# semihkacmaz/CoNFiLD

Measured on AMD Instinct MI355X. Metric: generated fields/sec (256-step sample + CNF decode), Case4 latent, 1/2/4/8 GPU, higher is better.
Workload: dtype f32

## Files before the change

confild_amd/csrc/siren.hip:

```cpp
#include <cmath>
#include <algorithm>
#include <cstdlib>
#include <cstring>
#include <string>
#include <type_traits>
#include <utility>
#include <vector>

#include "siren.hpp"

namespace cfd {

template <int NB, bool DUAL, int WAVES>
__global__ __launch_bounds__(64 * WAVES, (NB <= 24 && !DUAL) ? 2 : 1) void siren_fused(SirenArgs p) {
    constexpr int TILE = 16 * WAVES;
    constexpr int H = NB * 16;
    constexpr int BLK = NB * 256;
    extern __shared__ __attribute__((aligned(16))) float smem[];
    float* wbuf = smem;
    float* film = smem + 2 * BLK;

    const int lane = threadIdx.x & 63;
    const int wave = threadIdx.x >> 6;
    const int g = lane >> 4;
// ... 924 lines not shown
        case 12: return launch_siren_nb<12>(h, a, b, st);
        case 16: return launch_siren_nb<16>(h, a, b, st);
        case 24: return launch_siren_nb<24>(h, a, b, st);
        case 32: return launch_siren_nb<32>(h, a, b, st);
        default: throw cfd::Error{CFD_EARG, "hidden_features must be 16*{1,2,3,4,6,8,12,16,24,32}"};
    }
}

}

namespace {

void pack_split_f16(cfd_siren* h, int li, const float* W) {
    const int H = h->cfg.hidden_features, NB = h->NB, NQ = NB / 2;
    float amax = 0.f;
    for (size_t i = 0; i < (size_t)H * H; ++i) amax = std::max(amax, std::fabs(W[i]));
    int e = 0;
    if (amax > 0.f) std::frexp(amax, &e);
    const float s = std::ldexp(1.0f, -e);
    std::vector<_Float16> img((size_t)NB * NB * 512);
    for (int j = 0; j < NB; ++j)
        for (int q = 0; q < NQ; ++q)
            for (int l = 0; l < 64; ++l)
                for (int t = 0; t < 8; ++t) {
                    const float v = W[(size_t)(16 * j + l % 16) * H + 16 * (2 * q + t / 4) + 4 * (l / 16) + t % 4] * s;
                    const _Float16 hi = (_Float16)v;
                    const _Float16 lo = (_Float16)(v - (float)hi);
                    const size_t base = ((size_t)j * NB + 2 * q) * 512 + l * 8 + t;
                    img[base] = hi;
                    img[base + 512] = lo;
                }
    CFD_HIP(hipMemcpy(h->wimg16 + (size_t)(li - 1) * NB * NB * 256, img.data(), img.size() * sizeof(_Float16),
                      hipMemcpyHostToDevice));
    for (int j = 0; j < NB; ++j)
        for (int q = 0; q < NQ; ++q)
            for (int l = 0; l < 64; ++l)
                for (int t = 0; t < 8; ++t) {
                    const float v = W[(size_t)(16 * (2 * q + t / 4) + 4 * (l / 16) + t % 4) * H + 16 * j + l % 16] * s;
                    const _Float16 hi = (_Float16)v;
                    const _Float16 lo = (_Float16)(v - (float)hi);
                    const size_t base = ((size_t)j * NB + 2 * q) * 512 + l * 8 + t;
                    img[base] = hi;
                    img[base + 512] = lo;
                }
    CFD_HIP(hipMemcpy(h->wimg16t + (size_t)(h->cfg.num_hidden_layers - li) * NB * NB * 256, img.data(),
                      img.size() * sizeof(_Float16), hipMemcpyHostToDevice));
    if (H % 32 == 0) {
        const int NB2 = H / 32, NK = H / 16;
        for (int J = 0; J < NB2; ++J)
            for (int k = 0; k < NK; ++k)
                for (int l = 0; l < 64; ++l)
                    for (int t = 0; t < 8; ++t) {
                        const int jb = k / 2, e = k % 2;
                        const float v = W[(size_t)(32 * J + l % 32) * H + 32 * jb + 8 * (2 * e + t / 4) +
                                          4 * (l / 32) + t % 4] * s;
                        const _Float16 hi = (_Float16)v;
                        const _Float16 lo = (_Float16)(v - (float)hi);
                        const size_t base = ((size_t)J * NK + k) * 1024 + l * 8 + t;
                        img[base] = hi;
                        img[base + 512] = lo;
                    }
        CFD_HIP(hipMemcpy(h->wimg32 + (size_t)(li - 1) * NB * NB * 256, img.data(),
                          img.size() * sizeof(_Float16), hipMemcpyHostToDevice));
        const double kr = (double)h->cfg.w0 / (2.0 * M_PI);
        const double amr = (double)amax * kr;
        int er = 0;
        if (amr > 0.0) std::frexp(amr, &er);
        const double sr = std::ldexp(1.0, -er);
        for (int J = 0; J < NB2; ++J)
            for (int k = 0; k < NK; ++k)
                for (int l = 0; l < 64; ++l)
                    for (int t = 0; t < 8; ++t) {
                        const int jb = k / 2, e = k % 2;
                        const double v = (double)W[(size_t)(32 * J + l % 32) * H + 32 * jb + 8 * (2 * e + t / 4) +
                                                   4 * (l / 32) + t % 4] * kr * sr;
                        const _Float16 hi = (_Float16)v;
                        const _Float16 lo = (_Float16)(v - (double)hi);
                        const size_t base = ((size_t)J * NK + k) * 1024 + l * 8 + t;
                        img[base] = hi;
                        img[base + 512] = lo;
                    }
        CFD_HIP(hipMemcpy(h->wimg32r + (size_t)(li - 1) * NB * NB * 256, img.data(),
                          img.size() * sizeof(_Float16), hipMemcpyHostToDevice));
        const int nh = h->cfg.num_hidden_layers;
        const float fs = (float)(kr * sr), inv = (float)(1.0 / sr);
        CFD_HIP(hipMemcpy(h->wrev + (li - 1), &fs, sizeof(float), hipMemcpyHostToDevice));
        CFD_HIP(hipMemcpy(h->wrev + nh + (li - 1), &inv, sizeof(float), hipMemcpyHostToDevice));
    }
    CFD_HIP(hipMemcpy(h->wscale + (li - 1), &s, sizeof(float), hipMemcpyHostToDevice));
}

}

extern "C" int cfd_siren_create(const cfd_siren_cfg* cfg, int device, cfd_siren** out) {
    return cfd::guard([&] {
        CFD_REQUIRE(cfg && out, CFD_EARG, "null argument");
        const int d = cfg->in_coord_features, L = cfg->in_latent_features, c = cfg->out_features;
        const int nh = cfg->num_hidden_layers, H = cfg->hidden_features;
        CFD_REQUIRE(d >= 1 && d <= 4, CFD_EARG, "in_coord_features must be 1..4");
        CFD_REQUIRE(c >= 1 && c <= 4, CFD_EARG, "out_features must be 1..4");
        CFD_REQUIRE(L >= 1 && nh >= 0 && H % 16 == 0 && H >= 16 && H <= 512, CFD_EARG,
                    "hidden_features must be a multiple of 16 in [16, 512]");
        const int NB = H / 16;
        CFD_REQUIRE(NB == 1 || NB == 2 || NB == 3 || NB == 4 || NB == 6 || NB == 8 || NB == 12 || NB == 16 ||
                        NB == 24 || NB == 32,
                    CFD_EARG, "hidden_features must be 16*{1,2,3,4,6,8,12,16,24,32}");
        cfd::DeviceGuard dg(device);
        auto* h = new cfd_siren();
        h->cfg = *cfg;
        if (h->cfg.w0 == 0.f) h->cfg.w0 = 30.f;
        h->device = device;
        h->NB = NB;
        for (int i = 0; i < nh + 2; ++i) {
            const int fin = i == 0 ? d : H, fout = i == nh + 1 ? c : H;
            h->params.push_back({"net1." + std::to_string(i) + ".weight", {fout, fin}});
            h->params.push_back({"net1." + std::to_string(i) + ".bias", {fout}});
        }
        for (int i = 0; i < nh + 1; ++i) h->params.push_back({"net2." + std::to_string(i) + ".weight", {H, L}});
        CFD_HIP(hipMalloc(&h->w0, sizeof(float) * H * d));
        CFD_HIP(hipMalloc(&h->fbias, sizeof(float) * (nh + 1) * H));
        CFD_HIP(hipMalloc(&h->V, sizeof(float) * (size_t)(nh + 1) * H * L));
        CFD_HIP(hipMalloc(&h->wimg, sizeof(float) * (size_t)std::max(nh, 1) * NB * NB * 256));
        CFD_HIP(hipMalloc(&h->wout, sizeof(float) * c * H));
        CFD_HIP(hipMalloc(&h->bout, sizeof(float) * 4));
        CFD_HIP(hipMalloc(&h->wimg_t, sizeof(float) * (size_t)std::max(nh, 1) * NB * NB * 256));
        CFD_HIP(hipMalloc(&h->wimg16, sizeof(float) * (size_t)std::max(nh, 1) * NB * NB * 256));
        CFD_HIP(hipMalloc(&h->wimg16t, sizeof(float) * (size_t)std::max(nh, 1) * NB * NB * 256));
        CFD_HIP(hipMalloc(&h->wscale, sizeof(float) * (size_t)std::max(nh, 1)));
        CFD_HIP(hipMalloc(&h->wimg32, sizeof(float) * (size_t)std::max(nh, 1) * NB * NB * 256));
        CFD_HIP(hipMalloc(&h->wimg32r, sizeof(float) * (size_t)std::max(nh, 1) * NB * NB * 256));
        CFD_HIP(hipMalloc(&h->wrev, sizeof(float) * 2 * (size_t)std::max(nh, 1)));
        *out = h;
    });
}

extern "C" void cfd_siren_destroy(cfd_siren* h) {
    if (!h) return;
    (void)hipFree(h->w0);
    (void)hipFree(h->fbias);
    (void)hipFree(h->V);
    (void)hipFree(h->wimg);
    (void)hipFree(h->wout);
    (void)hipFree(h->bout);
    (void)hipFree(h->wimg_t);
    (void)hipFree(h->wimg16);
    (void)hipFree(h->wimg16t);
    (void)hipFree(h->wscale);
    (void)hipFree(h->wimg32);
    (void)hipFree(h->wimg32r);
    (void)hipFree(h->wrev);
    delete h;
}

extern "C" int cfd_siren_num_params(const cfd_siren* h, int* n) {
    return cfd::guard([&] {
        CFD_REQUIRE(h && n, CFD_EARG, "null argument");
        *n = (int)h->params.size();
    });
}

extern "C" int cfd_siren_param_info(const cfd_siren* h, int idx, const char** key, int* ndim, int64_t shape[4]) {
    return cfd::guard([&] {
        CFD_REQUIRE(h && idx >= 0 && idx < (int)h->params.size(), CFD_EARG, "bad index");
        const auto& p = h->params[idx];
        if (key) *key = p.key.c_str();
        if (ndim) *ndim = (int)p.shape.size();
        if (shape)
            for (size_t i = 0; i < p.shape.size(); ++i) shape[i] = p.shape[i];
    });
}

extern "C" int cfd_siren_set_param(cfd_siren* h, const char* key, const float* host, size_t n) {
    return cfd::guard([&] {
        CFD_REQUIRE(h && key && host, CFD_EARG, "null argument");
        cfd::DeviceGuard dg(h->device);
        const std::string k(key);
        cfd::SirenParam* prm = nullptr;
        for (auto& p : h->params)
            if (p.key == k) prm = &p;
        CFD_REQUIRE(prm, CFD_EKEY, "unknown SIREN parameter key: " + k);
        size_t want = 1;
        for (auto s : prm->shape) want *= (size_t)s;
        CFD_REQUIRE(n == want, CFD_ESHAPE, "size mismatch for " + k);
        const int d = h->cfg.in_coord_features, L = h->cfg.in_latent_features, c = h->cfg.out_features;
        const int nh = h->cfg.num_hidden_layers, H = h->cfg.hidden_features, NB = h->NB;
        const bool is_w = k.size() > 7 && k.compare(k.size() - 7, 7, ".weight") == 0;
        const int li = std::stoi(k.substr(5, k.find('.', 5) - 5));
        if (k.rfind("net2.", 0) == 0) {
            CFD_HIP(hipMemcpy(h->V + (size_t)li * H * L, host, n * 4, hipMemcpyHostToDevice));
        } else if (li == nh + 1) {
            CFD_HIP(hipMemcpy(is_w ? h->wout : h->bout, host, n * 4, hipMemcpyHostToDevice));
        } else if (!is_w) {
            CFD_HIP(hipMemcpy(h->fbias + (size_t)li * H, host, n * 4, hipMemcpyHostToDevice));
        } else if (li == 0) {
            CFD_HIP(hipMemcpy(h->w0, host, n * 4, hipMemcpyHostToDevice));
            (void)d;
        } else {
            std::vector<float> img((size_t)NB * NB * 256);
            for (int j = 0; j < NB; ++j)
                for (int q = 0; q < NB; ++q)
                    for (int lane = 0; lane < 64; ++lane)
                        for (int s = 0; s < 4; ++s)
                            img[(((size_t)j * NB + q) * 64 + lane) * 4 + s] =
                                host[(size_t)(16 * j + (lane & 15)) * H + 16 * q + 4 * (lane >> 4) + s];
            CFD_HIP(hipMemcpy(h->wimg + (size_t)(li - 1) * NB * NB * 256, img.data(), img.size() * 4,
                              hipMemcpyHostToDevice));
            for (int j = 0; j < NB; ++j)
                for (int q = 0; q < NB; ++q)
                    for (int lane = 0; lane < 64; ++lane)
                        for (int s2 = 0; s2 < 4; ++s2)
                            img[(((size_t)j * NB + q) * 64 + lane) * 4 + s2] =
                                host[(size_t)(16 * q + 4 * (lane >> 4) + s2) * H + 16 * j + (lane & 15)];
            CFD_HIP(hipMemcpy(h->wimg_t + (size_t)(nh - li) * NB * NB * 256, img.data(), img.size() * 4,
                              hipMemcpyHostToDevice));
            if (NB % 2 == 0) pack_split_f16(h, li, host);
        }
        (void)c;
        prm->set = true;
    });
}

extern "C" int cfd_siren_ready(const cfd_siren* h) {
    return cfd::guard([&] {
        CFD_REQUIRE(h, CFD_EARG, "null handle");
        for (const auto& p : h->params) CFD_REQUIRE(p.set, CFD_ESTATE, "SIREN parameter not set: " + p.key);
    });
}

extern "C" int cfd_siren_workspace_bytes(const cfd_siren* h, int b, size_t* bytes) {
    return cfd::guard([&] {
        CFD_REQUIRE(h && bytes && b >= 0, CFD_EARG, "bad argument");
        *bytes = sizeof(float) * (size_t)b * (h->cfg.num_hidden_layers + 1) * h->cfg.hidden_features;
    });
}

namespace cfd {
void film_vectors(const cfd_siren* h, const float* latents, int b, float* film, hipStream_t st) {
    const int nl = h->cfg.num_hidden_layers + 1, H = h->cfg.hidden_features, L = h->cfg.in_latent_features;
    if (L % 16 == 0) {
        cfd::launch_gemm_f32(true, latents, L, h->V, L, h->fbias, film, nl * H, b, nl * H, L, st);
        return;
    }
    hipLaunchKernelGGL(cfd::siren_film, dim3(nl, b), dim3(128), 0, st, h->V, h->fbias, latents, film, H, L, nl);
    cfd::check_launch("siren_film");
}
}
using cfd::film_vectors;

extern "C" int cfd_siren_forward(cfd_siren* h, const float* coords, int64_t N, const float* latents, int b,
                                 const float* xmax, const float* xmin, const float* ymax, const float* ymin,
                                 int64_t y_stride, float* out, void* ws, size_t ws_bytes, void* stream) {
    return cfd::guard([&] {
        CFD_REQUIRE(h && coords && latents && out, CFD_EARG, "null argument");
        CFD_REQUIRE(N >= 1 && b >= 1, CFD_EARG, "empty decode");
        CFD_REQUIRE((xmax == nullptr) == (xmin == nullptr), CFD_EARG, "xmax/xmin must both be set or both NULL");
        CFD_REQUIRE((ymax == nullptr) == (ymin == nullptr), CFD_EARG, "ymax/ymin must both be set or both NULL");
        size_t need = 0;
        cfd_siren_workspace_bytes(h, b, &need);
        CFD_REQUIRE(ws && ws_bytes >= need, CFD_EARG, "workspace too small");
        const int nh = h->cfg.num_hidden_layers, H = h->cfg.hidden_features;
        auto st = (hipStream_t)stream;
        float* film = (float*)ws;
        film_vectors(h, latents, b, film, st);
        cfd::SirenArgs a{};
        a.w0 = h->w0;
        a.wimg = h->wimg;
        a.wout = h->wout;
        a.bout = h->bout;
        a.film = film;
        a.coords = coords;
        a.xmax = xmax;
        a.xmin = xmin;
        a.ymax = ymax;
        a.ymin = ymin;
        a.out = out;
        a.N = N;
        a.ystride = y_stride;
        a.d = h->cfg.in_coord_features;
        a.c = h->cfg.out_features;
        a.nh = nh;
        a.stamps = cfd::stamps_buf();
        a.w0f = h->cfg.w0;
        if (h->compute == CFD_SIREN_SPLIT_F16 && nh >= 1 && cfd::siren_split_supported(h->NB)) {
            a.wscale = h->wscale;
            if (cfd::siren_split32_supported(H, nh)) {
                a.wimg = h->wimg32;
                a.wimg_rev = h->wimg32r;
                a.wrev = h->wrev;
                cfd::launch_siren_split32(H, a, b, st);
            } else {
                a.wimg = h->wimg16;
                cfd::launch_siren_split(h->NB, a, b, st);
            }
        } else {
            launch_siren(h, a, b, st);
        }
    });
}

extern "C" int cfd_siren_set_compute(cfd_siren* h, int compute) {
    return cfd::guard([&] {
        CFD_REQUIRE(h, CFD_EARG, "null handle");
        CFD_REQUIRE(compute == CFD_SIREN_F32 || compute == CFD_SIREN_SPLIT_F16, CFD_EARG, "unknown SIREN compute mode");
        h->compute = compute;
    });
}

extern "C" int cfd_siren_get_compute(const cfd_siren* h, int* compute) {
    return cfd::guard([&] {
        CFD_REQUIRE(h && compute, CFD_EARG, "null argument");
        const bool split = h->compute == CFD_SIREN_SPLIT_F16 && h->cfg.num_hidden_layers >= 1 &&
                           cfd::siren_split_supported(h->NB);
        *compute = split ? CFD_SIREN_SPLIT_F16 : CFD_SIREN_F32;
    });
}

namespace {

void tape_args(const cfd_siren* h, cfd::SirenTapeArgs& a, int64_t Ns, int R, void* ws) {
    const int nh = h->cfg.num_hidden_layers, H = h->cfg.hidden_features;
    const size_t nl = nh + 1;
    a.w0 = h->w0;
    a.wimg = h->wimg;
    a.wimg_t = h->wimg_t;
    a.wout = h->wout;
    a.bout = h->bout;
    a.film = (float*)ws;
    a.u = (float*)ws + (size_t)R * nl * H;
    a.delta = a.u + (size_t)R * Ns * nl * H;
    a.P = (int64_t)R * Ns;
    a.Ns = (int)Ns;
    a.d = h->cfg.in_coord_features;
    a.c = h->cfg.out_features;
    a.nh = nh;
    a.w0f = h->cfg.w0;
    if (h->compute == CFD_SIREN_SPLIT_F16 && nh >= 1 && cfd::tape_split_supported(h->NB)) {
        a.wimg16 = h->wimg16;
        a.wimg16t = h->wimg16t;
        a.wscale = h->wscale;
    }
}

int tape_waves(int64_t P) { return P >= 16 * 4 * 512 ? 4 : P >= 16 * 2 * 256 ? 2 : 1; }

template <int NB, int W>
void launch_tape_w(const cfd::SirenTapeArgs& a, bool bwd, hipStream_t st) {
    const size_t lds = sizeof(float) * (2 * NB * 256 + (bwd ? 0 : 4 * NB * 16));
    const void* fn = bwd ? (const void*)cfd::siren_tape_bwd<NB, W> : (const void*)cfd::siren_tape_fwd<NB, W>;
    CFD_HIP(hipFuncSetAttribute(fn, hipFuncAttributeMaxDynamicSharedMemorySize, (int)lds));
    const dim3 grid((unsigned)cfd::ceil_div(a.P, 16 * W));
    if (bwd)
        hipLaunchKernelGGL((cfd::siren_tape_bwd<NB, W>), grid, dim3(64 * W), lds, st, a);
    else
        hipLaunchKernelGGL((cfd::siren_tape_fwd<NB, W>), grid, dim3(64 * W), lds, st, a);
    cfd::check_launch(bwd ? "siren_tape_bwd" : "siren_tape_fwd");
}

template <int NB, int KS>
void launch_tape_ks(const cfd::SirenTapeArgs& a, bool bwd, hipStream_t st) {
    const size_t lds = sizeof(float) * (2 * NB * 256 + 2 * KS * 256 + (bwd ? 0 : 4 * NB * 16 + KS * 64));
    const void* fn = bwd ? (const void*)cfd::siren_tape_bwd_ks<NB, KS> : (const void*)cfd::siren_tape_fwd_ks<NB, KS>;
    CFD_HIP(hipFuncSetAttribute(fn, hipFuncAttributeMaxDynamicSharedMemorySize, (int)lds));
    const dim3 grid((unsigned)cfd::ceil_div(a.P, 16));
    if (bwd)
        hipLaunchKernelGGL((cfd::siren_tape_bwd_ks<NB, KS>), grid, dim3(64 * KS), lds, st, a);
    else
        hipLaunchKernelGGL((cfd::siren_tape_fwd_ks<NB, KS>), grid, dim3(64 * KS), lds, st, a);
    cfd::check_launch(bwd ? "siren_tape_bwd_ks" : "siren_tape_fwd_ks");
}

// ... 243 lines not shown
```

confild_amd/csrc/siren.hpp:

```cpp
#pragma once
#include <string>
#include <type_traits>
#include <utility>
#include <vector>

#include "common.hpp"

namespace cfd {

template <int N, class F, int... I>
__device__ __forceinline__ void static_for_impl(F&& f, std::integer_sequence<int, I...>) {
    (f(std::integral_constant<int, I>{}), ...);
}
template <int N, class F>
__device__ __forceinline__ void static_for(F&& f) {
    static_for_impl<N>(f, std::make_integer_sequence<int, N>{});
}

struct SirenArgs {
    const float* w0;
    const float* wimg;
    const float* wout;
    const float* bout;
    const float* film;
    const float* coords;
    const float* xmax;
    const float* xmin;
    const float* ymax;
    const float* ymin;
    float* out;
    const float* wscale;
    const float* wimg_rev;
    const float* wrev;
    int64_t N;
    int64_t ystride;
    int64_t b0;
    int d, c, nh;
    float w0f;
    unsigned long long* stamps;
};
struct SirenTapeArgs {
    const float* w0;
    const float* wimg;
    const float* wimg_t;
    const float* wout;
    const float* bout;
    const float* film;
    const float* coords;
    const float* xmax;
    const float* xmin;
    const float* ymax;
    const float* ymin;
    float* u;
    float* delta;
    float* out;
    const float* gout;
    const float* wimg16;
    const float* wimg16t;
    const float* wscale;
    int64_t P;
    int64_t ystride;
    int Ns, d, c, nh;
    float w0f;
};
unsigned long long* stamps_buf();

template <int NB, int WAVES>
__device__ __forceinline__ void siren_issue_block(const float* __restrict__ wimg, int J, float* dst,
                                                  int wave, int lane) {
    constexpr int BLK = NB * 256;
    const float* src = wimg + (int64_t)__builtin_amdgcn_readfirstlane(J) * BLK;
    for (int piece = wave; piece < NB; piece += WAVES) {
        __builtin_amdgcn_global_load_lds((const void*)(src + piece * 256 + lane * 4),
                                         (__attribute__((address_space(3))) void*)(dst + piece * 256),
                                         16, 0, 0);
    }
}

template <int NB, int WAVES>
__device__ __forceinline__ void siren_issue_block_u(const float* __restrict__ wimg, int J, float* dst,
                                                    int wave, int lane) {
    static_assert(NB % WAVES == 0, "whole pieces per wave");
    constexpr int BLK = NB * 256;
    const float* src = wimg + (int64_t)__builtin_amdgcn_readfirstlane(J) * BLK;
    static_for<NB / WAVES>([&](auto mc) {
        constexpr int m = decltype(mc)::value;
        const int piece = wave + m * WAVES;
        __builtin_amdgcn_global_load_lds((const void*)(src + piece * 256 + lane * 4),
                                         (__attribute__((address_space(3))) void*)(dst + piece * 256), 16, 0, 0);
    });
}

bool siren_split_supported(int NB);
void launch_siren_split(int NB, SirenArgs a, int b, hipStream_t st);
bool siren_split32_supported(int H, int nh);
void launch_siren_split32(int H, SirenArgs a, int b, hipStream_t st);
bool tape_split_supported(int NB);
void launch_tape_split(int NB, const SirenTapeArgs& a, bool bwd, hipStream_t st);
void launch_tape_split_sum(int NB, const SirenTapeArgs& a, int rows, hipStream_t st);

struct SirenParam {
    std::string key;
    std::vector<int64_t> shape;
    bool set = false;
};

}

struct cfd_siren {
    cfd_siren_cfg cfg;
    int device = 0;
    int NB = 0;
    std::vector<cfd::SirenParam> params;
    float* w0 = nullptr;
    float* fbias = nullptr;
    float* V = nullptr;
    float* wimg = nullptr;
    float* wout = nullptr;
    float* bout = nullptr;
    float* wimg_t = nullptr;
    float* wimg16 = nullptr;
    float* wimg16t = nullptr;
    float* wscale = nullptr;
    float* wimg32 = nullptr;
    float* wimg32r = nullptr;
    float* wrev = nullptr;
    int compute = CFD_SIREN_SPLIT_F16;
    int dense_bwd = CFD_DENSE_BWD_SUM;
    int dense_compute = CFD_DENSE_COMPUTE_AUTO;
};

namespace cfd {

int gemm_splits(int K);
void launch_gemm_f32(bool bt, const float* A, int lda, const float* B, int ldb, const float* bias, float* C, int ldc,
                     int M, int N, int K, hipStream_t st, float* part = nullptr);
void film_vectors(const cfd_siren* h, const float* latents, int b, float* film, hipStream_t st);

}
```

confild_amd/csrc/siren_split.hip:

```cpp
#include <cstdint>
#include <cstdlib>
#include <algorithm>

#include "siren.hpp"

typedef _Float16 h8 __attribute__((ext_vector_type(8)));
typedef _Float16 h2 __attribute__((ext_vector_type(2)));
typedef float f2 __attribute__((ext_vector_type(2)));
typedef unsigned u2 __attribute__((ext_vector_type(2)));
typedef unsigned u4 __attribute__((ext_vector_type(4)));

namespace cfd {

struct Frag {
    u4 v;
    __device__ __forceinline__ h8 h() const { return __builtin_bit_cast(h8, v); }
};

__device__ __forceinline__ unsigned pk_f16(float a, float b) {
    return __builtin_bit_cast(unsigned, __builtin_convertvector((f2){a, b}, h2));
}

__device__ __forceinline__ void split8(const float (&x0)[4], const float (&x1)[4], Frag& hi, Frag& lo) {
    unsigned hw[4], lw[4];
// ... 252 lines not shown
                for (int c = 0; c < CG; ++c)
                    a[c] = __builtin_amdgcn_mfma_f32_16x16x32_f16(FL[q], BH[c][q].h(), a[c], 0, 0, 0);
#pragma unroll
                for (int c = 0; c < CG; ++c)
                    a[c] = __builtin_amdgcn_mfma_f32_16x16x32_f16(FH[q], BL[c][q].h(), a[c], 0, 0, 0);
#pragma unroll
                for (int c = 0; c < CG; ++c)
                    a[c] = __builtin_amdgcn_mfma_f32_16x16x32_f16(FH[q], BH[c][q].h(), a[c], 0, 0, 0);
                if constexpr (j > 0) {
                    if constexpr (q == 0) sines(prev);
                    if constexpr (q == QE) epilogue(std::integral_constant<int, j - 1>{});
                }
                __builtin_amdgcn_sched_barrier(0);
            });
#pragma unroll
            for (int c = 0; c < CG; ++c) prev[c] = a[c];
            if constexpr (j % RB == RB - 1) {
                if (NOSYNC) {
                } else if (steady) {
                    if (PC_HI == PC_LO || !pc_hi)
                        __builtin_amdgcn_s_waitcnt(vmcnt_imm((RING - 2) * PC_LO));
                    else
                        __builtin_amdgcn_s_waitcnt(vmcnt_imm((RING - 2) * PC_HI));
                } else {
                    __builtin_amdgcn_s_waitcnt(vmcnt_imm(0));
                }
                if (!NOSYNC) asm volatile("s_barrier" ::: "memory");
                ++J;
                slot = slot == RING - 1 ? 0 : slot + 1;
            }
        });
        sines(prev);
        epilogue(std::integral_constant<int, NB - 1>{});
        static_for<NQ>([&](auto qc) {
            constexpr int q = decltype(qc)::value;
#pragma unroll
            for (int c = 0; c < CG; ++c) {
                BH[c][q] = NH[c][q];
                BL[c][q] = NL[c][q];
            }
        });
    }

#pragma unroll
    for (int c = 0; c < CG; ++c) {
        float ov[4];
#pragma unroll
        for (int oc = 0; oc < 4; ++oc) {
            float sum = o[c][oc];
            sum += __shfl_xor(sum, 16);
            sum += __shfl_xor(sum, 32);
            ov[oc] = oc < p.c ? sum + p.bout[oc] : 0.f;
        }
        const int64_t n = n0 + 16 * c;
        if (n < p.N && g < p.c) {
            float v = g == 0 ? ov[0] : g == 1 ? ov[1] : g == 2 ? ov[2] : ov[3];
            if (p.ymax) {
                const int64_t yi = n * p.ystride + g;
                const float hi = p.ymax[yi], lo = p.ymin[yi];
                v = (v + 1.0f) / 2.0f * (hi - lo) + lo;
            }
            p.out[(b * p.N + n) * p.c + g] = v;
        }
    }
}

typedef float f16v __attribute__((ext_vector_type(16)));

__device__ __forceinline__ void split2_mix(float a, float b, unsigned& hi, unsigned& lo) {
    hi = pk_f16(a, b);
    asm("v_fma_mixlo_f16 %0, %1, 1.0, -%2 op_sel_hi:[0,0,1]" : "=&v"(lo) : "v"(a), "v"(hi));
    asm("v_fma_mixhi_f16 %0, %1, 1.0, -%2 op_sel:[0,0,1] op_sel_hi:[0,0,1]" : "+v"(lo) : "v"(b), "v"(hi));
}

__device__ __forceinline__ void split_chunk(const float (&x)[16], int e, Frag& hi, Frag& lo) {
    unsigned hw[4], lw[4];
#pragma unroll
    for (int w = 0; w < 4; ++w) split2_mix(x[8 * e + 2 * w], x[8 * e + 2 * w + 1], hw[w], lw[w]);
    hi.v = (u4){hw[0], hw[1], hw[2], hw[3]};
    lo.v = (u4){lw[0], lw[1], lw[2], lw[3]};
    asm volatile("" : "+v"(hi.v), "+v"(lo.v));
}

template <int NB2, int EXP = 0, int HWSIN = 0>
__global__ __launch_bounds__(256, 1) void siren_split32(SirenArgs p) {
    constexpr int NK = 2 * NB2;
    constexpr int H = 32 * NB2;
    constexpr int BLK = NK * 512;
    constexpr int WAVES = 4, TILE = 128;
    constexpr int NPC = 2 * NK;
    constexpr int PPW = NPC / WAVES;
    constexpr int NKS = NK >= 18 ? 16 : NK - 2;
    extern __shared__ __attribute__((aligned(16))) float smem[];
    const int nh = p.nh;
    float* wbuf = smem;
    float* film = smem + 2 * BLK;
    float* w0s = film + (nh + 1) * H;
    float* wos = w0s + 4 * H;

    const int lane = threadIdx.x & 63;
    const int wave = __builtin_amdgcn_readfirstlane(threadIdx.x >> 6);
    const int h = lane >> 5;
    const int64_t b = p.b0 + blockIdx.y;
    const int64_t n = (int64_t)blockIdx.x * TILE + wave * 32 + (lane & 31);
    CFD_DASSERT(p.d >= 1 && p.d <= 4 && p.c >= 1 && p.c <= 4 && nh >= 1);
#ifdef CFD_STAMPS
    const bool stamped = blockIdx.x % 61 == 0;
    if (stamped) CFD_STAMP(p.stamps, 5, (unsigned)blockIdx.y, 0);
    __builtin_amdgcn_s_waitcnt(0xC07F);
#endif

    {
        const float* fsrc = p.film + b * (int64_t)(nh + 1) * H;
        const int nf = (nh + 1) * H;
        for (int i = threadIdx.x * 4; i < nf; i += 64 * WAVES * 4) {
            const int layer = i / H;
            const float sc = layer == 0 ? 1.0f : HWSIN >= 3 ? p.wrev[layer - 1] : p.wscale[layer - 1];
            *(f4*)(film + i) = *(const f4*)(fsrc + i) * sc;
        }
    }
    for (int f = threadIdx.x; f < H; f += 64 * WAVES) {
        f4 w = {0.f, 0.f, 0.f, 0.f};
        for (int k = 0; k < p.d; ++k) w[k] = p.w0[f * p.d + k];
        *(f4*)(w0s + 4 * f) = w;
    }
    for (int i = threadIdx.x; i < 4 * H; i += 64 * WAVES) wos[i] = i < p.c * H ? p.wout[i] : 0.f;
    float cn[4];
    {
        const int64_t nc = n < p.N ? n : p.N - 1;
#pragma unroll
        for (int k = 0; k < 4; ++k) {
            float v = 0.f;
            if (k < p.d) {
                v = p.coords[nc * p.d + k];
                if (p.xmax) v = (v - p.xmin[k]) / (p.xmax[k] - p.xmin[k]) * 2.0f - 1.0f;
            }
            cn[k] = v;
        }
    }
    __syncthreads();
    const int nblocks = nh * NB2;
    const __amdgpu_buffer_rsrc_t wrsrc =
        __builtin_amdgcn_make_buffer_rsrc((void*)p.wimg, 0, nblocks * (BLK * 4), 0x00020000);
    siren_issue_block<NPC, WAVES>(p.wimg, 0, wbuf, wave, lane);

    Frag BH[NK], BL[NK], NH[NK], NL[NK];
    float o[4] = {0.f, 0.f, 0.f, 0.f};

    static_for<NB2>([&](auto Jc) {
        constexpr int J = decltype(Jc)::value;
        float x[16];
#pragma unroll
        for (int qq = 0; qq < 4; ++qq) {
            const f4 fv = *(const f4*)(film + 32 * J + 8 * qq + 4 * h);
#pragma unroll
            for (int r = 0; r < 4; ++r) {
                const f4 w = *(const f4*)(w0s + 4 * (32 * J + 8 * qq + 4 * h + r));
                float a = cn[0] * w[0];
#pragma unroll
                for (int k = 1; k < 4; ++k)
                    if (k < p.d) a = fmaf(cn[k], w[k], a);
                x[4 * qq + r] = hidden_sine<HWSIN >= 2 ? 2 : HWSIN>(p.w0f * (a + fv[r]));
            }
        }
        split_chunk(x, 0, NH[2 * J], NL[2 * J]);
        split_chunk(x, 1, NH[2 * J + 1], NL[2 * J + 1]);
    });

    static_assert(NB2 % 2 == 0, "static ring slots need an even block count");
    int J = 0;
    f16v prev;
    float mprev = 0.f;
    float x[16];
    h8 FH, FL;
    f16v an;
    auto film_row = [&](const float* frow) __attribute__((always_inline)) {
#pragma unroll
        for (int qq = 0; qq < 4; ++qq) {
            const f4 f = *(const f4*)(frow + 8 * qq + 4 * h);
#pragma unroll
            for (int r = 0; r < 4; ++r) an[4 * qq + r] = f[r];
        }
    };
    if constexpr (!(EXP & 1)) {
        __builtin_amdgcn_s_waitcnt(vmcnt_imm(0));
        asm volatile("s_barrier" ::: "memory");
    }
    FH = *(const h8*)(wbuf + lane * 4);
    FL = *(const h8*)(wbuf + 256 + lane * 4);
    for (int layer = 1; layer <= nh; ++layer) {
        const bool last = layer == nh;
        const float m = HWSIN >= 3 ? p.wrev[nh + layer - 1] : p.w0f / p.wscale[layer - 1];
        auto outsum = [&](int jp, int e) __attribute__((always_inline)) {
            const int f = 32 * jp + 8 * e + 4 * h;
#pragma unroll
            for (int oc = 0; oc < 4; ++oc) {
                const f4 w = *(const f4*)(wos + oc * H + f);
#pragma unroll
                for (int r = 0; r < 4; ++r) o[oc] = fmaf(w[r], x[4 * e + r], o[oc]);
            }
        };
        static_for<NB2>([&](auto jc) {
            constexpr int j = decltype(jc)::value;
            constexpr int jp = j == 0 ? NB2 - 1 : j - 1;
            const float me = j == 0 ? mprev : m;
            const bool live = j > 0 || layer > 1;
            float* nxt = wbuf + ((j & 1) ^ 1) * BLK;
            const float* wb = wbuf + (j & 1) * BLK;
            const int soff = __builtin_amdgcn_readfirstlane(min(J + 1, nblocks - 1)) * (BLK * 4);
            if constexpr (j == 0) film_row(film + layer * H);
            f16v a = an;
            static_for<NK>([&](auto kc) {
                constexpr int k = decltype(kc)::value;
                h8 FH1 = FH, FL1 = FL;
                if constexpr (k + 1 < NK && !(EXP & 4)) {
                    FH1 = *(const h8*)(wb + (k + 1) * 512 + lane * 4);
                    FL1 = *(const h8*)(wb + (k + 1) * 512 + 256 + lane * 4);
                }
                if constexpr (k == NK - 1) {
                    if constexpr (j + 1 < NB2) film_row(film + layer * H + 32 * (j + 1));
                    FH1 = *(const h8*)(nxt + lane * 4);
                    FL1 = *(const h8*)(nxt + 256 + lane * 4);
                }
                if constexpr (k < PPW && !(EXP & 1)) {
                    const int piece = wave + WAVES * k;
                    __builtin_amdgcn_raw_ptr_buffer_load_lds(
                        wrsrc, (__attribute__((address_space(3))) void*)(nxt + piece * 256), 16, lane * 16,
                        soff + piece * 1024, 0, 0);
                }
                if constexpr (j == 0) {
                    a = __builtin_amdgcn_mfma_f32_32x32x16_f16(FL, NH[k].h(), a, 0, 0, 0);
                    a = __builtin_amdgcn_mfma_f32_32x32x16_f16(FH, NL[k].h(), a, 0, 0, 0);
                    a = __builtin_amdgcn_mfma_f32_32x32x16_f16(FH, NH[k].h(), a, 0, 0, 0);
                    BH[k] = NH[k];
                    BL[k] = NL[k];
                    asm volatile("" : "+a"(BH[k].v), "+a"(BL[k].v));
                } else {
                    a = __builtin_amdgcn_mfma_f32_32x32x16_f16(FL, BH[k].h(), a, 0, 0, 0);
                    a = __builtin_amdgcn_mfma_f32_32x32x16_f16(FH, BL[k].h(), a, 0, 0, 0);
                    a = __builtin_amdgcn_mfma_f32_32x32x16_f16(FH, BH[k].h(), a, 0, 0, 0);
                }
                if constexpr (k < NKS) {
#pragma unroll
                    for (int v = 16 * k / NKS; v < 16 * (k + 1) / NKS; ++v) {
                        x[v] = (EXP & 2) ? prev[v] * me : hidden_sine<HWSIN>(prev[v] * me);
                        asm volatile("" : "+v"(x[v]));
                    }
                }
                constexpr int KE = NK >= 18 ? 16 : NKS - 1;
                if constexpr (k == KE || k == (NK >= 18 ? 17 : KE)) {
                    constexpr bool both = NK < 18;
                    constexpr int e0 = (NK >= 18 && k == 17) ? 1 : 0;
                    if (live) {
#pragma unroll
                        for (int e = e0; e < (both ? 2 : e0 + 1); ++e)
                            split_chunk(x, e, NH[2 * jp + e], NL[2 * jp + e]);
                        if (j > 0 && last) {
#pragma unroll
                            for (int e = 2 * e0; e < (both ? 4 : 2 * e0 + 2); ++e) outsum(jp, e);
                        }
                    }
                }
                __builtin_amdgcn_sched_barrier(0);
                FH = FH1;
                FL = FL1;
                if constexpr (k == NK - 2 && !(EXP & 1)) {
                    __builtin_amdgcn_s_waitcnt(vm_lgkm0_imm(0));
                    asm volatile("s_barrier" ::: "memory");
                    __builtin_amdgcn_sched_barrier(0);
                }
            });
            prev = a;
            ++J;
        });
        mprev = m;
    }
#pragma unroll
    for (int v = 0; v < 16; ++v) x[v] = hidden_sine<HWSIN>(prev[v] * mprev);
    {
        const int f0 = 32 * (NB2 - 1) + 4 * h;
#pragma unroll
        for (int e = 0; e < 4; ++e)
#pragma unroll
            for (int oc = 0; oc < 4; ++oc) {
                const f4 w = *(const f4*)(wos + oc * H + f0 + 8 * e);
#pragma unroll
                for (int r = 0; r < 4; ++r) o[oc] = fmaf(w[r], x[4 * e + r], o[oc]);
            }
    }

    float ov[4];
#pragma unroll
    for (int oc = 0; oc < 4; ++oc) {
        const float sum = o[oc] + __shfl_xor(o[oc], 32);
        ov[oc] = oc < p.c ? sum + p.bout[oc] : 0.f;
    }
    if (n < p.N) {
#pragma unroll
        for (int i = 0; i < 2; ++i) {
            const int oc = 2 * h + i;
            if (oc < p.c) {
                float v = ov[oc];
                if (p.ymax) {
                    const int64_t yi = n * p.ystride + oc;
                    const float hi = p.ymax[yi], lo = p.ymin[yi];
                    v = (v + 1.0f) / 2.0f * (hi - lo) + lo;
                }
                p.out[(b * p.N + n) * p.c + oc] = v;
            }
        }
    }
#ifdef CFD_STAMPS
    if (stamped) CFD_STAMP(p.stamps, 5, (unsigned)blockIdx.y, 4);
#endif
}

namespace {

template <int NB, int RING, int CG, int RB = 1, bool NOSYNC = false, bool PKSIN = true>
void launch_ring(SirenArgs a, int b, hipStream_t st) {
    constexpr int H = NB * 16;
    constexpr int WAVES = CG == 1 ? 8 : 4;
    const size_t lds = sizeof(float) * ((size_t)RING * RB * NB * 256 + (size_t)(a.nh + 1) * H + 8 * H);
    const void* fn = (const void*)siren_fused_split<NB, WAVES, RING, CG, RB, NOSYNC, PKSIN>;
    CFD_REQUIRE(lds <= 160 * 1024, CFD_EARG, "SIREN too deep for the split-f16 decoder's LDS staging");
    CFD_HIP(hipFuncSetAttribute(fn, hipFuncAttributeMaxDynamicSharedMemorySize, (int)lds));
    const int64_t tiles = ceil_div(a.N, 16 * CG * WAVES);
    CFD_REQUIRE(tiles <= 0x7fffffff, CFD_EARG, "too many coordinates for one launch");
    for (int64_t b0 = 0; b0 < b; b0 += 65535) {
        a.b0 = b0;
        const int nb = (int)std::min<int64_t>(65535, b - b0);
        hipLaunchKernelGGL((siren_fused_split<NB, WAVES, RING, CG, RB, NOSYNC, PKSIN>), dim3((unsigned)tiles, nb),
                           dim3(64 * WAVES), lds, st, a);
        check_launch("siren_fused_split");
    }
}

template <int NB>
void launch_nb(SirenArgs a, int b, hipStream_t st) {
    launch_ring<NB, 2, 1, 1>(a, b, st);
}
}

template <int NB2, int EXP = 0, int HWSIN = 0>
void launch_split32(SirenArgs a, int b, hipStream_t st) {
    constexpr int H = NB2 * 32;
    const size_t lds = sizeof(float) * ((size_t)2 * 2 * NB2 * 512 + (size_t)(a.nh + 1) * H + 8 * H);
    const void* fn = (const void*)siren_split32<NB2, EXP, HWSIN>;
    CFD_REQUIRE((int64_t)a.nh * H * H * 4 < 0x7fffffffLL, CFD_EARG, "weight image beyond the 2 GiB buffer range");
    CFD_REQUIRE(lds <= 160 * 1024, CFD_EARG, "SIREN too deep for the split-f16 decoder's LDS staging");
    CFD_HIP(hipFuncSetAttribute(fn, hipFuncAttributeMaxDynamicSharedMemorySize, (int)lds));
    const int64_t tiles = ceil_div(a.N, 128);
    CFD_REQUIRE(tiles <= 0x7fffffff, CFD_EARG, "too many coordinates for one launch");
    for (int64_t b0 = 0; b0 < b; b0 += 65535) {
        a.b0 = b0;
        const int nb = (int)std::min<int64_t>(65535, b - b0);
        hipLaunchKernelGGL((siren_split32<NB2, EXP, HWSIN>), dim3((unsigned)tiles, nb), dim3(256), lds, st, a);
        check_launch("siren_split32");
    }
}

bool siren_split32_supported(int H, int nh) {
    const size_t film = (size_t)(nh + 1) * H + 8 * (size_t)H;
    return (H == 64 || H == 128 || H == 256 || H == 384) &&
           sizeof(float) * ((size_t)4 * (H / 32) * 512 + film) <= 160 * 1024;
}

void launch_siren_split32(int H, SirenArgs a, int b, hipStream_t st) {
    CFD_REQUIRE(a.wimg_rev && a.wrev, CFD_EARG, "split32 revolution image not set");
    a.wimg = a.wimg_rev;
    switch (H) {
        case 64: return launch_split32<2, 0, 4>(a, b, st);
        case 128: return launch_split32<4, 0, 4>(a, b, st);
        case 256: return launch_split32<8, 0, 4>(a, b, st);
        case 384: return launch_split32<12, 0, 4>(a, b, st);
        default: throw Error{CFD_EARG, "32x32 split-f16 SIREN needs hidden_features in {64, 128, 256, 384}"};
    }
}

bool siren_split_supported(int NB) {
    switch (NB) {
        case 2: case 4: case 6: case 8: case 12: case 16: case 24: return true;
        default: return false;
    }
}

void launch_siren_split(int NB, SirenArgs a, int b, hipStream_t st) {
    switch (NB) {
        case 2: return launch_nb<2>(a, b, st);
        case 4: return launch_nb<4>(a, b, st);
        case 6: return launch_nb<6>(a, b, st);
        case 8: return launch_nb<8>(a, b, st);
        case 12: return launch_nb<12>(a, b, st);
        case 16: return launch_nb<16>(a, b, st);
        case 24: return launch_nb<24>(a, b, st);
        default: throw Error{CFD_EARG, "split-f16 SIREN needs hidden_features = 32*{1,2,3,4,6,8,12,16}"};
    }
}

template <int NB, int KS, int RING>
__global__ __launch_bounds__(64 * KS) void siren_tape_fwd_split(SirenTapeArgs p) {
    constexpr int H = NB * 16, BLK = NB * 256, QW = NB / KS, QC = QW / 2;
    static_assert(QW % 2 == 0 && (RING == 2 || RING == 3), "K9t: an even block count per wave");
    extern __shared__ __attribute__((aligned(16))) float smem[];
    float* wbuf = smem;
    float* red = smem + RING * BLK;
    const int lane = threadIdx.x & 63;
    const int wave = __builtin_amdgcn_readfirstlane(threadIdx.x >> 6);
    const int g = lane >> 4, j16 = lane & 15;
    const int64_t n = (int64_t)blockIdx.x * 16 + j16;
    const int64_t nc = n < p.P ? n : p.P - 1;
    const int64_t row = nc / p.Ns;
    const int sensor = (int)(nc - row * p.Ns);
    const int nh = p.nh, nl = nh + 1;
    const float* film = p.film + row * nl * H;
    float* ut = p.u + nc * nl * H;
    const int q0 = wave * QW;
    const int nblocks = nh * NB;

    float cn[4] = {0.f, 0.f, 0.f, 0.f};
#pragma unroll
    for (int k = 0; k < 4; ++k) {
        if (k < p.d) {
            float v = p.coords[(int64_t)sensor * p.d + k];
            if (p.xmax) v = (v - p.xmin[k]) / (p.xmax[k] - p.xmin[k]) * 2.0f - 1.0f;
            cn[k] = v;
        }
    }
#pragma unroll
    for (int r = 0; r + 1 < RING; ++r)
        if (r < nblocks) siren_issue_block_u<NB, KS>(p.wimg16, r, wbuf + r * BLK, wave, lane);

    float X[QW][4], Xn[QW][4];
    static_for<QW>([&](auto qc) {
        constexpr int qq = decltype(qc)::value;
        const int q = q0 + qq;
        const f4 fv = *(const f4*)(film + 16 * q + 4 * g);
        f4 uu;
#pragma unroll
        for (int r = 0; r < 4; ++r) {
            const float* w = p.w0 + (16 * q + 4 * g + r) * p.d;
            float a = cn[0] * w[0];
#pragma unroll
            for (int k = 1; k < 4; ++k)
                if (k < p.d) a = fmaf(cn[k], w[k], a);
            uu[r] = a + fv[r];
            X[qq][r] = sin_cw(p.w0f * uu[r]);
        }
        *(f4*)(ut + 16 * q + 4 * g) = uu;
    });
    Frag xh[QC], xl[QC];
    auto split_x = [&]() __attribute__((always_inline)) {
        static_for<QC>([&](auto ic) {
            constexpr int i = decltype(ic)::value;
            split8(X[2 * i], X[2 * i + 1], xh[i], xl[i]);
        });
    };
    split_x();
// ... 392 lines not shown
```

Before: 3.978.

## Add 16x16x32 MFMA variant of split-f16 SIREN decoder with matching weight image

Adds a new kernel body that computes the split-f16 SIREN hidden layers using 16x16x32 f16 MFMA tiles instead of the 32x32 shape. It also builds a second weight image laid out for that fragment shape, and makes it the default for hidden widths 128/256/384. Each wave handles two 16-point column groups, so the weight fragment is reused across them. The sine and split work is interleaved across the k-steps. The aim is better MFMA throughput and latency hiding in the decoder. The cost is an extra weight buffer, a more complex register schedule, and possible register pressure.

```diff
diff --git a/confild_amd/csrc/siren.hip b/confild_amd/csrc/siren.hip
--- a/confild_amd/csrc/siren.hip
+++ b/confild_amd/csrc/siren.hip
@@ -1030,6 +1030,21 @@
                     }
         CFD_HIP(hipMemcpy(h->wimg32r + (size_t)(li - 1) * NB * NB * 256, img.data(),
                           img.size() * sizeof(_Float16), hipMemcpyHostToDevice));
+        for (int J = 0; J < NB2; ++J)
+            for (int k = 0; k < NK; ++k)
+                for (int l = 0; l < 64; ++l)
+                    for (int t = 0; t < 8; ++t) {
+                        const int q = k / 2, rb = k % 2;
+                        const double v = (double)W[(size_t)(32 * J + 16 * rb + l % 16) * H + 16 * (2 * q + t / 4) +
+                                                   4 * (l / 16) + t % 4] * kr * sr;
+                        const _Float16 hi = (_Float16)v;
+                        const _Float16 lo = (_Float16)(v - (double)hi);
+                        const size_t base = ((size_t)J * NK + k) * 1024 + l * 8 + t;
+                        img[base] = hi;
+                        img[base + 512] = lo;
+                    }
+        CFD_HIP(hipMemcpy(h->wimg16r + (size_t)(li - 1) * NB * NB * 256, img.data(),
+                          img.size() * sizeof(_Float16), hipMemcpyHostToDevice));
         const int nh = h->cfg.num_hidden_layers;
         const float fs = (float)(kr * sr), inv = (float)(1.0 / sr);
         CFD_HIP(hipMemcpy(h->wrev + (li - 1), &fs, sizeof(float), hipMemcpyHostToDevice));
@@ -1078,6 +1093,7 @@
         CFD_HIP(hipMalloc(&h->wimg32, sizeof(float) * (size_t)std::max(nh, 1) * NB * NB * 256));
         CFD_HIP(hipMalloc(&h->wimg32r, sizeof(float) * (size_t)std::max(nh, 1) * NB * NB * 256));
         CFD_HIP(hipMalloc(&h->wrev, sizeof(float) * 2 * (size_t)std::max(nh, 1)));
+        CFD_HIP(hipMalloc(&h->wimg16r, sizeof(float) * (size_t)std::max(nh, 1) * NB * NB * 256));
         *out = h;
     });
 }
@@ -1097,6 +1113,7 @@
     (void)hipFree(h->wimg32);
     (void)hipFree(h->wimg32r);
     (void)hipFree(h->wrev);
+    (void)hipFree(h->wimg16r);
     delete h;
 }
 
@@ -1234,6 +1251,7 @@
             if (cfd::siren_split32_supported(H, nh)) {
                 a.wimg = h->wimg32;
                 a.wimg_rev = h->wimg32r;
+                a.wimg_rev16 = h->wimg16r;
                 a.wrev = h->wrev;
                 cfd::launch_siren_split32(H, a, b, st);
             } else {
diff --git a/confild_amd/csrc/siren.hpp b/confild_amd/csrc/siren.hpp
--- a/confild_amd/csrc/siren.hpp
+++ b/confild_amd/csrc/siren.hpp
@@ -32,6 +32,7 @@
     const float* wscale;
     const float* wimg_rev;
     const float* wrev;
+    const float* wimg_rev16;
     int64_t N;
     int64_t ystride;
     int64_t b0;
@@ -125,6 +126,7 @@
     float* wimg32 = nullptr;
     float* wimg32r = nullptr;
     float* wrev = nullptr;
+    float* wimg16r = nullptr;
     int compute = CFD_SIREN_SPLIT_F16;
     int dense_bwd = CFD_DENSE_BWD_SUM;
     int dense_compute = CFD_DENSE_COMPUTE_AUTO;
diff --git a/confild_amd/csrc/siren_split.hip b/confild_amd/csrc/siren_split.hip
--- a/confild_amd/csrc/siren_split.hip
+++ b/confild_amd/csrc/siren_split.hip
@@ -358,8 +358,14 @@
     asm volatile("" : "+v"(hi.v), "+v"(lo.v));
 }
 
-template <int NB2, int EXP = 0, int HWSIN = 0>
-__global__ __launch_bounds__(256, 1) void siren_split32(SirenArgs p) {
+__device__ __forceinline__ float fma_scalar(float a, float b, float c) {
+    float d;
+    asm("v_fma_f32 %0, %1, %2, %3" : "=v"(d) : "v"(a), "v"(b), "v"(c));
+    return d;
+}
+
+template <int NB2, int EXP, int HWSIN>
+__device__ __forceinline__ void split32_body(const SirenArgs& p) {
     constexpr int NK = 2 * NB2;
     constexpr int H = 32 * NB2;
     constexpr int BLK = NK * 512;
@@ -473,7 +479,7 @@
             for (int oc = 0; oc < 4; ++oc) {
                 const f4 w = *(const f4*)(wos + oc * H + f);
 #pragma unroll
-                for (int r = 0; r < 4; ++r) o[oc] = fmaf(w[r], x[4 * e + r], o[oc]);
+                for (int r = 0; r < 4; ++r) o[oc] = fma_scalar(w[r], x[4 * e + r], o[oc]);
             }
         };
         static_for<NB2>([&](auto jc) {
@@ -591,6 +597,272 @@
 #endif
 }
 
+template <int NB2, int EXP, int HWSIN>
+__device__ __forceinline__ void split16_body(const SirenArgs& p) {
+    constexpr int NQ = NB2;
+    constexpr int NK = 2 * NB2;
+    constexpr int H = 32 * NB2;
+    constexpr int BLK = NK * 512;
+    constexpr int WAVES = 4, TILE = 128;
+    constexpr int NPC = 2 * NK;
+    constexpr int PPW = NPC / WAVES;
+    constexpr int NKS = NK >= 18 ? 16 : NK - 2;
+    extern __shared__ __attribute__((aligned(16))) float smem[];
+    const int nh = p.nh;
+    float* wbuf = smem;
+    float* film = smem + 2 * BLK;
+    float* w0s = film + (nh + 1) * H;
+    float* wos = w0s + 4 * H;
+
+    const int lane = threadIdx.x & 63;
+    const int wave = __builtin_amdgcn_readfirstlane(threadIdx.x >> 6);
+    const int g = lane >> 4;
+    const int64_t b = p.b0 + blockIdx.y;
+    const int64_t n0 = (int64_t)blockIdx.x * TILE + wave * 32 + (lane & 15);
+    CFD_DASSERT(p.d >= 1 && p.d <= 4 && p.c >= 1 && p.c <= 4 && nh >= 1);
+#ifdef CFD_STAMPS
+    const bool stamped = blockIdx.x % 61 == 0;
+    if (stamped) CFD_STAMP(p.stamps, 5, (unsigned)blockIdx.y, 0);
+    __builtin_amdgcn_s_waitcnt(0xC07F);
+#endif
+
+    {
+        const float* fsrc = p.film + b * (int64_t)(nh + 1) * H;
+        const int nf = (nh + 1) * H;
+        for (int i = threadIdx.x * 4; i < nf; i += 64 * WAVES * 4) {
+            const int layer = i / H;
+            const float sc = layer == 0 ? 1.0f : HWSIN >= 3 ? p.wrev[layer - 1] : p.wscale[layer - 1];
+            *(f4*)(film + i) = *(const f4*)(fsrc + i) * sc;
+        }
+    }
+    for (int f = threadIdx.x; f < H; f += 64 * WAVES) {
+        f4 w = {0.f, 0.f, 0.f, 0.f};
+        for (int k = 0; k < p.d; ++k) w[k] = p.w0[f * p.d + k];
+        *(f4*)(w0s + 4 * f) = w;
+    }
+    for (int i = threadIdx.x; i < 4 * H; i += 64 * WAVES) wos[i] = i < p.c * H ? p.wout[i] : 0.f;
+    float cn[2][4];
+#pragma unroll
+    for (int c = 0; c < 2; ++c) {
+        const int64_t n = n0 + 16 * c;
+        const int64_t nc = n < p.N ? n : p.N - 1;
+#pragma unroll
+        for (int k = 0; k < 4; ++k) {
+            float v = 0.f;
+            if (k < p.d) {
+                v = p.coords[nc * p.d + k];
+                if (p.xmax) v = (v - p.xmin[k]) / (p.xmax[k] - p.xmin[k]) * 2.0f - 1.0f;
+            }
+            cn[c][k] = v;
+        }
+    }
+    __syncthreads();
+    const int nblocks = nh * NB2;
+    const __amdgpu_buffer_rsrc_t wrsrc =
+        __builtin_amdgcn_make_buffer_rsrc((void*)p.wimg, 0, nblocks * (BLK * 4), 0x00020000);
+    siren_issue_block<NPC, WAVES>(p.wimg, 0, wbuf, wave, lane);
+
+    Frag BH[NK], BL[NK], NH[NK], NL[NK];
+    float o[2][4] = {{0.f, 0.f, 0.f, 0.f}, {0.f, 0.f, 0.f, 0.f}};
+
+    static_for<NB2>([&](auto Jc) {
+        constexpr int J = decltype(Jc)::value;
+        float x[16];
+#pragma unroll
+        for (int rb = 0; rb < 2; ++rb) {
+            const f4 fv = *(const f4*)(film + 32 * J + 16 * rb + 4 * g);
+#pragma unroll
+            for (int r = 0; r < 4; ++r) {
+                const f4 w = *(const f4*)(w0s + 4 * (32 * J + 16 * rb + 4 * g + r));
+#pragma unroll
+                for (int c = 0; c < 2; ++c) {
+                    float a = cn[c][0] * w[0];
+#pragma unroll
+                    for (int k = 1; k < 4; ++k)
+                        if (k < p.d) a = fmaf(cn[c][k], w[k], a);
+                    x[8 * c + 4 * rb + r] = hidden_sine<HWSIN >= 2 ? 2 : HWSIN>(p.w0f * (a + fv[r]));
+                }
+            }
+        }
+        split_chunk(x, 0, NH[J], NL[J]);
+        split_chunk(x, 1, NH[NQ + J], NL[NQ + J]);
+    });
+
+    static_assert(NB2 % 2 == 0, "static ring slots need an even block count");
+    int J = 0;
+    float prev[16];
+#pragma unroll
+    for (int v = 0; v < 16; ++v) prev[v] = 0.f;
+    float mprev = 0.f;
+    float x[16];
+    h8 FH, FL;
+    f4 an[2][2];
+    int g1 = g;
+    asm volatile("" : "+v"(g1));
+    auto film_row = [&](const float* frow) __attribute__((always_inline)) {
+#pragma unroll
+        for (int rb = 0; rb < 2; ++rb) {
+            an[rb][0] = *(const f4*)(frow + 16 * rb + 4 * g);
+            an[rb][1] = *(const f4*)(frow + 16 * rb + 4 * g1);
+        }
+    };
+    if constexpr (!(EXP & 1)) {
+        __builtin_amdgcn_s_waitcnt(vmcnt_imm(0));
+        asm volatile("s_barrier" ::: "memory");
+    }
+    FH = *(const h8*)(wbuf + lane * 4);
+    FL = *(const h8*)(wbuf + 256 + lane * 4);
+    for (int layer = 1; layer <= nh; ++layer) {
+        const bool last = layer == nh;
+        const float m = HWSIN >= 3 ? p.wrev[nh + layer - 1] : p.w0f / p.wscale[layer - 1];
+        auto outsum = [&](int jp, int c, int rb) __attribute__((always_inline)) {
+            const int f = 32 * jp + 16 * rb + 4 * g;
+#pragma unroll
+            for (int oc = 0; oc < 4; ++oc) {
+                const f4 w = *(const f4*)(wos + oc * H + f);
+#pragma unroll
+                for (int r = 0; r < 4; ++r) o[c][oc] = fma_scalar(w[r], x[8 * c + 4 * rb + r], o[c][oc]);
+            }
+        };
+        static_for<NB2>([&](auto jc) {
+            constexpr int j = decltype(jc)::value;
+            constexpr int jp = j == 0 ? NB2 - 1 : j - 1;
+            const float me = j == 0 ? mprev : m;
+            const bool live = j > 0 || layer > 1;
+            float* nxt = wbuf + ((j & 1) ^ 1) * BLK;
+            const float* wb = wbuf + (j & 1) * BLK;
+            const int soff = __builtin_amdgcn_readfirstlane(min(J + 1, nblocks - 1)) * (BLK * 4);
+            if constexpr (j == 0) film_row(film + layer * H);
+            f4 acc[2][2];
+#pragma unroll
+            for (int rb = 0; rb < 2; ++rb)
+#pragma unroll
+                for (int c = 0; c < 2; ++c) acc[rb][c] = an[rb][c];
+            static_for<NK>([&](auto kc) {
+                constexpr int k = decltype(kc)::value;
+                constexpr int q = k / 2, rb = k % 2;
+                h8 FH1 = FH, FL1 = FL;
+                if constexpr (k + 1 < NK && !(EXP & 4)) {
+                    FH1 = *(const h8*)(wb + (k + 1) * 512 + lane * 4);
+                    FL1 = *(const h8*)(wb + (k + 1) * 512 + 256 + lane * 4);
+                }
+                if constexpr (k == NK - 1) {
+                    if constexpr (j + 1 < NB2) film_row(film + layer * H + 32 * (j + 1));
+                    FH1 = *(const h8*)(nxt + lane * 4);
+                    FL1 = *(const h8*)(nxt + 256 + lane * 4);
+                }
+                if constexpr (k < PPW && !(EXP & 1)) {
+                    const int piece = wave + WAVES * k;
+                    __builtin_amdgcn_raw_ptr_buffer_load_lds(
+                        wrsrc, (__attribute__((address_space(3))) void*)(nxt + piece * 256), 16, lane * 16,
+                        soff + piece * 1024, 0, 0);
+                }
+                if constexpr (j == 0) {
+                    acc[rb][0] = __builtin_amdgcn_mfma_f32_16x16x32_f16(FL, NH[q].h(), acc[rb][0], 0, 0, 0);
+                    acc[rb][1] = __builtin_amdgcn_mfma_f32_16x16x32_f16(FL, NH[NQ + q].h(), acc[rb][1], 0, 0, 0);
+                    acc[rb][0] = __builtin_amdgcn_mfma_f32_16x16x32_f16(FH, NL[q].h(), acc[rb][0], 0, 0, 0);
+                    acc[rb][1] = __builtin_amdgcn_mfma_f32_16x16x32_f16(FH, NL[NQ + q].h(), acc[rb][1], 0, 0, 0);
+                    acc[rb][0] = __builtin_amdgcn_mfma_f32_16x16x32_f16(FH, NH[q].h(), acc[rb][0], 0, 0, 0);
+                    acc[rb][1] = __builtin_amdgcn_mfma_f32_16x16x32_f16(FH, NH[NQ + q].h(), acc[rb][1], 0, 0, 0);
+                    BH[rb * NQ + q] = NH[rb * NQ + q];
+                    BL[rb * NQ + q] = NL[rb * NQ + q];
+                    asm volatile("" : "+a"(BH[rb * NQ + q].v), "+a"(BL[rb * NQ + q].v));
+                } else {
+                    acc[rb][0] = __builtin_amdgcn_mfma_f32_16x16x32_f16(FL, BH[q].h(), acc[rb][0], 0, 0, 0);
+                    acc[rb][1] = __builtin_amdgcn_mfma_f32_16x16x32_f16(FL, BH[NQ + q].h(), acc[rb][1], 0, 0, 0);
+                    acc[rb][0] = __builtin_amdgcn_mfma_f32_16x16x32_f16(FH, BL[q].h(), acc[rb][0], 0, 0, 0);
+                    acc[rb][1] = __builtin_amdgcn_mfma_f32_16x16x32_f16(FH, BL[NQ + q].h(), acc[rb][1], 0, 0, 0);
+                    acc[rb][0] = __builtin_amdgcn_mfma_f32_16x16x32_f16(FH, BH[q].h(), acc[rb][0], 0, 0, 0);
+                    acc[rb][1] = __builtin_amdgcn_mfma_f32_16x16x32_f16(FH, BH[NQ + q].h(), acc[rb][1], 0, 0, 0);
+                }
+                if constexpr (k < NKS) {
+#pragma unroll
+                    for (int v = 16 * k / NKS; v < 16 * (k + 1) / NKS; ++v) {
+                        x[v] = (EXP & 2) ? prev[v] * me : hidden_sine<HWSIN>(prev[v] * me);
+                        asm volatile("" : "+v"(x[v]));
+                    }
+                }
+                constexpr int KE = NK >= 18 ? 16 : NKS - 1;
+                if constexpr (k == KE || k == (NK >= 18 ? 17 : KE)) {
+                    constexpr bool both = NK < 18;
+                    constexpr int c0 = (NK >= 18 && k == 17) ? 1 : 0;
+                    if (live) {
+#pragma unroll
+                        for (int c = c0; c < (both ? 2 : c0 + 1); ++c)
+                            split_chunk(x, c, NH[c * NQ + jp], NL[c * NQ + jp]);
+                        if (j > 0 && last) {
+#pragma unroll
+                            for (int c = c0; c < (both ? 2 : c0 + 1); ++c) {
+                                outsum(jp, c, 0);
+                                outsum(jp, c, 1);
+                            }
+                        }
+                    }
+                }
+                __builtin_amdgcn_sched_barrier(0);
+                FH = FH1;
+                FL = FL1;
+                if constexpr (k == NK - 2 && !(EXP & 1)) {
+                    __builtin_amdgcn_s_waitcnt(vm_lgkm0_imm(0));
+                    asm volatile("s_barrier" ::: "memory");
+                    __builtin_amdgcn_sched_barrier(0);
+                }
+            });
+#pragma unroll
+            for (int rb = 0; rb < 2; ++rb)
+#pragma unroll
+                for (int c = 0; c < 2; ++c)
+#pragma unroll
+                    for (int r = 0; r < 4; ++r) prev[8 * c + 4 * rb + r] = acc[rb][c][r];
+            ++J;
+        });
+        mprev = m;
+    }
+#pragma unroll
+    for (int v = 0; v < 16; ++v) x[v] = hidden_sine<HWSIN>(prev[v] * mprev);
+#pragma unroll
+    for (int rb = 0; rb < 2; ++rb)
+#pragma unroll
+        for (int oc = 0; oc < 4; ++oc) {
+            const f4 w = *(const f4*)(wos + oc * H + 32 * (NB2 - 1) + 16 * rb + 4 * g);
+#pragma unroll
+            for (int c = 0; c < 2; ++c)
+#pragma unroll
+                for (int r = 0; r < 4; ++r) o[c][oc] = fmaf(w[r], x[8 * c + 4 * rb + r], o[c][oc]);
+        }
+
+#pragma unroll
+    for (int c = 0; c < 2; ++c) {
+        float ov[4];
+#pragma unroll
+        for (int oc = 0; oc < 4; ++oc) {
+            float sum = o[c][oc];
+            sum += __shfl_xor(sum, 16);
+            sum += __shfl_xor(sum, 32);
+            ov[oc] = oc < p.c ? sum + p.bout[oc] : 0.f;
+        }
+        const int64_t n = n0 + 16 * c;
+        if (n < p.N && g < p.c) {
+            float v = g == 0 ? ov[0] : g == 1 ? ov[1] : g == 2 ? ov[2] : ov[3];
+            if (p.ymax) {
+                const int64_t yi = n * p.ystride + g;
+                const float hi = p.ymax[yi], lo = p.ymin[yi];
+                v = (v + 1.0f) / 2.0f * (hi - lo) + lo;
+            }
+            p.out[(b * p.N + n) * p.c + g] = v;
+        }
+    }
+#ifdef CFD_STAMPS
+    if (stamped) CFD_STAMP(p.stamps, 5, (unsigned)blockIdx.y, 4);
+#endif
+}
+
+template <int NB2, int EXP = 0, int HWSIN = 0, int SHAPE = 32>
+__global__ __launch_bounds__(256, 1) void siren_split32(SirenArgs p) {
+    if constexpr (SHAPE == 16) split16_body<NB2, EXP, HWSIN>(p);
+    else split32_body<NB2, EXP, HWSIN>(p);
+}
+
 namespace {
 
 template <int NB, int RING, int CG, int RB = 1, bool NOSYNC = false, bool PKSIN = true>
@@ -618,11 +890,11 @@
 }
 }
 
-template <int NB2, int EXP = 0, int HWSIN = 0>
+template <int NB2, int EXP = 0, int HWSIN = 0, int SHAPE = 32>
 void launch_split32(SirenArgs a, int b, hipStream_t st) {
     constexpr int H = NB2 * 32;
     const size_t lds = sizeof(float) * ((size_t)2 * 2 * NB2 * 512 + (size_t)(a.nh + 1) * H + 8 * H);
-    const void* fn = (const void*)siren_split32<NB2, EXP, HWSIN>;
+    const void* fn = (const void*)siren_split32<NB2, EXP, HWSIN, SHAPE>;
     CFD_REQUIRE((int64_t)a.nh * H * H * 4 < 0x7fffffffLL, CFD_EARG, "weight image beyond the 2 GiB buffer range");
     CFD_REQUIRE(lds <= 160 * 1024, CFD_EARG, "SIREN too deep for the split-f16 decoder's LDS staging");
     CFD_HIP(hipFuncSetAttribute(fn, hipFuncAttributeMaxDynamicSharedMemorySize, (int)lds));
@@ -631,9 +903,23 @@
     for (int64_t b0 = 0; b0 < b; b0 += 65535) {
         a.b0 = b0;
         const int nb = (int)std::min<int64_t>(65535, b - b0);
-        hipLaunchKernelGGL((siren_split32<NB2, EXP, HWSIN>), dim3((unsigned)tiles, nb), dim3(256), lds, st, a);
+        hipLaunchKernelGGL((siren_split32<NB2, EXP, HWSIN, SHAPE>), dim3((unsigned)tiles, nb), dim3(256), lds, st, a);
         check_launch("siren_split32");
     }
+}
+
+#ifdef CFD_SPLIT32_SHAPE
+constexpr int SHAPE_64 = CFD_SPLIT32_SHAPE, SHAPE_128 = CFD_SPLIT32_SHAPE, SHAPE_256 = CFD_SPLIT32_SHAPE,
+              SHAPE_384 = CFD_SPLIT32_SHAPE;
+#else
+constexpr int SHAPE_64 = 32, SHAPE_128 = 16, SHAPE_256 = 16, SHAPE_384 = 16;
+#endif
+static_assert((SHAPE_64 == 16 || SHAPE_64 == 32) && (SHAPE_384 == 16 || SHAPE_384 == 32), "the shape define takes 16 or 32");
+
+template <int NB2, int SHAPE>
+void launch_split32_shape(SirenArgs a, int b, hipStream_t st) {
+    a.wimg = SHAPE == 16 ? a.wimg_rev16 : a.wimg_rev;
+    launch_split32<NB2, 0, 4, SHAPE>(a, b, st);
 }
 
 bool siren_split32_supported(int H, int nh) {
@@ -643,13 +929,12 @@
 }
 
 void launch_siren_split32(int H, SirenArgs a, int b, hipStream_t st) {
-    CFD_REQUIRE(a.wimg_rev && a.wrev, CFD_EARG, "split32 revolution image not set");
-    a.wimg = a.wimg_rev;
+    CFD_REQUIRE(a.wimg_rev && a.wimg_rev16 && a.wrev, CFD_EARG, "split32 revolution images not set");
     switch (H) {
-        case 64: return launch_split32<2, 0, 4>(a, b, st);
-        case 128: return launch_split32<4, 0, 4>(a, b, st);
-        case 256: return launch_split32<8, 0, 4>(a, b, st);
-        case 384: return launch_split32<12, 0, 4>(a, b, st);
+        case 64: return launch_split32_shape<2, SHAPE_64>(a, b, st);
+        case 128: return launch_split32_shape<4, SHAPE_128>(a, b, st);
+        case 256: return launch_split32_shape<8, SHAPE_256>(a, b, st);
+        case 384: return launch_split32_shape<12, SHAPE_384>(a, b, st);
         default: throw Error{CFD_EARG, "32x32 split-f16 SIREN needs hidden_features in {64, 128, 256, 384}"};
     }
 }
```

Measured after the change: 4.094, median of 6. 2.9% higher.
